# nanoporetech/medaka

Measured on NVIDIA H100. Metric: pileup positions/sec (consensus inference), higher is better.
Workload: dtype f32

## Files before the change

### medaka_b200/csrc/gru_wg.cu

```cuda
#include "common.cuh"
#include "ptx.cuh"
#include "rec_common.cuh"

namespace mdk {

constexpr int RW_THREADS = 256;
constexpr int RW_ABLK = (H / 8) * 64 * 16;
constexpr int RW_XBLK = 2 * 64 * 16;

template <int NT, bool FUSE_X, int OUT>
struct RwCfg {
    static constexpr int N = NT * RT_N;
    static constexpr bool HL = NT == 1;
    static constexpr int ROWS = HL ? 2 * N : N;
    static constexpr int PLANES = HL ? 1 : 2;
    static constexpr int KG = ROWS * 16 + 16;
    static constexpr int HPLANE = (H / 8) * KG;
    static constexpr int XPLANE = 2 * KG;
    static constexpr int HLO = HL ? N * 16 : HPLANE;
    static constexpr int XLO = HL ? N * 16 : XPLANE;
    static constexpr int RED = (RW_THREADS / 32) * NCLS * N;
    static constexpr int wlo_off = 0;
    static constexpr int wxlo_off = wlo_off + 6 * RW_ABLK;
    static constexpr int h_off = wxlo_off + (FUSE_X ? 6 * RW_XBLK : 0);
    static constexpr int x_off = h_off + 2 * PLANES * HPLANE;
    static constexpr int red_off = x_off + (FUSE_X ? 2 * PLANES * XPLANE : 0);
    static constexpr int total = red_off + (OUT == OUT_LOGITS ? 2 * RED * 4 : 0);
    static_assert(total <= 227 * 1024, "smem budget");
};

__device__ __forceinline__ uint32_t ld_u32(const __half *p) { return *reinterpret_cast<const uint32_t *>(p); }

template <int NT, bool FUSE_X, int OUT>
__global__ void __launch_bounds__(RW_THREADS, 1)
rec_tc_kernel(const float *__restrict__ gi, RecX xin, const __half *__restrict__ w_hh, const float *__restrict__ b_hn,
              void *__restrict__ h_out, int64_t B, int64_t T, const float *__restrict__ lin_w,
              float *__restrict__ plog) {
    using L = RwCfg<NT, FUSE_X, OUT>;
    constexpr int N = L::N, NA = N / 2;
    constexpr int NACC = L::ROWS / 2;
    constexpr int NX = FUSE_X ? NACC : NA;
    using MMA = Wgmma<N>;
    using MMA_H = Wgmma<L::ROWS>;
    constexpr bool LOGITS = OUT == OUT_LOGITS;
    extern __shared__ __align__(128) uint8_t smem[];
    const int tid = threadIdx.x, wg = tid >> 7, warp = (tid >> 5) & 3, lane = tid & 31;
    const int gq = lane >> 2, cq = lane & 3;
    const int dir = blockIdx.y;
    const int64_t ntiles = (B + RT_N - 1) / RT_N;
    const int64_t wtile0 = (int64_t)blockIdx.x * NT;
    const int j0 = wg * 64 + warp * 16 + gq;
    const uint32_t sbase = smem_u32(smem);

    for (int i = tid; i < (L::total - L::h_off) / 16; i += RW_THREADS)
        reinterpret_cast<int4 *>(smem + L::h_off)[i] = make_int4(0, 0, 0, 0);
    for (int i = tid; i < 3 * H * (H / 8); i += RW_THREADS) {
        const int kg = i & 15, r = (i >> 4) & (H - 1), gate = i >> 11;
        const uint4 v = *reinterpret_cast<const uint4 *>(w_hh + ((((size_t)dir * 2 + 1) * 3 + gate) * H + r) * H + kg * 8);
        *reinterpret_cast<uint4 *>(smem + L::wlo_off + (gate * 2 + (r >> 6)) * RW_ABLK + kg * 1024 + (r & 63) * 16) = v;
    }
    if (FUSE_X) {
        for (int i = tid; i < 3 * H * 2; i += RW_THREADS) {
            const int kg = i & 1, r = (i >> 1) & (H - 1), gate = i >> 8;
            const uint4 v = *reinterpret_cast<const uint4 *>(xin.w_x + ((((size_t)dir * 2 + 1) * 3 + gate) * H + r) * 16 + kg * 8);
            *reinterpret_cast<uint4 *>(smem + L::wxlo_off + (gate * 2 + (r >> 6)) * RW_XBLK + kg * 1024 + (r & 63) * 16) = v;
        }
    }
    float wlin[2][NCLS];
    if (LOGITS) {
#pragma unroll
        for (int hb = 0; hb < 2; ++hb)
#pragma unroll
            for (int c = 0; c < NCLS; ++c) wlin[hb][c] = lin_w[c * H2 + dir * H + j0 + 8 * hb];
    }
    uint32_t whi[3][H / 16][4];
#pragma unroll
    for (int gate = 0; gate < 3; ++gate)
#pragma unroll
        for (int ks = 0; ks < H / 16; ++ks) {
            const __half *w = w_hh + ((((size_t)dir * 2) * 3 + gate) * H + j0) * H + ks * 16 + 2 * cq;
            whi[gate][ks][0] = ld_u32(w);
            whi[gate][ks][1] = ld_u32(w + 8 * H);
            whi[gate][ks][2] = ld_u32(w + 8);
            whi[gate][ks][3] = ld_u32(w + 8 * H + 8);
        }
    uint32_t wxhi[3][4];
    float bx[3][2] = {};
    if (FUSE_X) {
#pragma unroll
        for (int gate = 0; gate < 3; ++gate) {
            const __half *w = xin.w_x + ((((size_t)dir * 2) * 3 + gate) * H + j0) * 16 + 2 * cq;
            wxhi[gate][0] = ld_u32(w);
            wxhi[gate][1] = ld_u32(w + 8 * 16);
            wxhi[gate][2] = ld_u32(w + 8);
            wxhi[gate][3] = ld_u32(w + 8 * 16 + 8);
            bx[gate][0] = xin.bias[dir * G3 + gate * H + j0];
            bx[gate][1] = xin.bias[dir * G3 + gate * H + j0 + 8];
        }
    }
    const float bhn[2] = {b_hn[dir * H + j0], b_hn[dir * H + j0 + 8]};

    float ar[NACC], az[NACC], an[NACC], axn[NX], hp[NA];
#pragma unroll
    for (int k = 0; k < NA; ++k) hp[k] = 0.f;
    auto load_pre = [&](int64_t t) {
#pragma unroll
        for (int i = 0; i < N / 8; ++i)
#pragma unroll
            for (int hb = 0; hb < 2; ++hb) {
                float2 v[3] = {make_float2(0.f, 0.f), make_float2(0.f, 0.f), make_float2(0.f, 0.f)};
                if (FUSE_X) {
#pragma unroll
                    for (int gate = 0; gate < 3; ++gate) v[gate] = make_float2(bx[gate][hb], bx[gate][hb]);
                } else if (wtile0 + (i >> 1) < ntiles) {
                    const float *p = gi + ((wtile0 + (i >> 1)) * T + t) * GI_TS_FLOATS +
                                     (((dir * 3) * 4 + 2 * (i & 1) + (cq >> 1)) * H + j0 + 8 * hb) * 4 + 2 * (cq & 1);
#pragma unroll
                    for (int gate = 0; gate < 3; ++gate) v[gate] = __ldcs(reinterpret_cast<const float2 *>(p + gate * 16 * H));
                }
                const int k = 4 * i + 2 * hb;
                ar[k] = v[0].x; ar[k + 1] = v[0].y;
                az[k] = v[1].x; az[k + 1] = v[1].y;
                axn[k] = v[2].x; axn[k + 1] = v[2].y;
                an[k] = bhn[hb]; an[k + 1] = bhn[hb];
            }
        if constexpr (L::HL) {
#pragma unroll
            for (int k = NA; k < NACC; ++k) {
                ar[k] = 0.f; az[k] = 0.f; an[k] = 0.f;
                if constexpr (FUSE_X) axn[k] = 0.f;
            }
        }
    };
    const int xF = FUSE_X ? xin.F : 1;
    const float *xsrc[NT];
    int xoff[NT];
    float xreg[NT];
#pragma unroll
    for (int m = 0; m < NT; ++m) {
        const int q = tid + RW_THREADS * m, xn = q / xF, xf = q - xn * xF;
        const bool own = FUSE_X && q < N * xF;
        xoff[m] = own ? (xf >> 3) * L::KG + xn * 16 + (xf & 7) * 2 : -1;
        xsrc[m] = (own && wtile0 * RT_N + xn < B) ? xin.feats + ((wtile0 * RT_N + xn) * T) * xF + xf : nullptr;
        xreg[m] = 0.f;
    }
    auto stage_x = [&](int buf, int m, float v) {
        __half hi, lo;
        split_f16(v, hi, lo);
        *reinterpret_cast<__half *>(smem + L::x_off + buf * L::PLANES * L::XPLANE + xoff[m]) = hi;
        *reinterpret_cast<__half *>(smem + L::x_off + buf * L::PLANES * L::XPLANE + L::XLO + xoff[m]) = lo;
    };
    const int64_t t_first = dir ? T - 1 : 0;
    if (FUSE_X) {
#pragma unroll
        for (int m = 0; m < NT; ++m) {
            if (xoff[m] < 0) continue;
            stage_x(0, m, xsrc[m] ? xsrc[m][t_first * xF] : 0.f);
            if (xsrc[m] && T > 1) xreg[m] = xsrc[m][(dir ? T - 2 : 1) * xF];
        }
    }
    load_pre(t_first);
    fence_proxy_async_smem();
    __syncthreads();

    constexpr int NW = N / 4;
    auto head_partials = [&](int rb) {
        float v[NW][NCLS];
#pragma unroll
        for (int wl = 0; wl < NW; ++wl) {
            const int k = 4 * (wl >> 1) + (wl & 1);
#pragma unroll
            for (int c = 0; c < NCLS; ++c) v[wl][c] = fmaf(wlin[1][c], hp[k + 2], wlin[0][c] * hp[k]);
        }
        int wbase = 0;
#pragma unroll
        for (int lvl = 0; lvl < 3; ++lvl) {
            const int mask = 16 >> lvl;
            const int half = (NW >> lvl) / 2;
            if (half > 0) {
                const bool up = lane & mask;
#pragma unroll
                for (int w = 0; w < NW / 2; ++w) {
                    if (w >= half) continue;
#pragma unroll
                    for (int c = 0; c < NCLS; ++c) {
                        const float send = up ? v[w][c] : v[w + half][c];
                        const float keep = up ? v[w + half][c] : v[w][c];
                        v[w][c] = keep + __shfl_xor_sync(0xffffffffu, send, mask);
                    }
                }
                if (up) wbase += half;
            } else {
#pragma unroll
                for (int c = 0; c < NCLS; ++c) v[0][c] += __shfl_xor_sync(0xffffffffu, v[0][c], mask);
            }
        }
        if (NW >= 8 || !(lane & 4)) {
            float *red = reinterpret_cast<float *>(smem + L::red_off) + rb * L::RED + (tid >> 5) * NCLS * N;
            const int n = 8 * (wbase >> 1) + 2 * cq + (wbase & 1);
#pragma unroll
            for (int c = 0; c < NCLS; ++c) red[c * N + n] = v[0][c];
        }
    };
    auto head_store = [&](int rb, int64_t t) {
        if (tid >= NCLS * N) return;
        const int c = tid / N, n = tid % N;
        const float *red = reinterpret_cast<const float *>(smem + L::red_off) + rb * L::RED + c * N + n;
        float s = red[0];
#pragma unroll
        for (int w = 1; w < RW_THREADS / 32; ++w) s += red[w * NCLS * N];
        const int64_t wt = wtile0 + n / RT_N;
        if (wt < ntiles) plog[((dir * ntiles + wt) * T + t) * PLOG_TS_FLOATS + c * RT_N + (n & 15)] = s;
    };

#pragma unroll 1
    for (int64_t step = 0; step < T; ++step) {
        const int64_t t = dir ? T - 1 - step : step;
        const int buf = (int)(step & 1);
        const uint32_t hb_addr = sbase + L::h_off + buf * L::PLANES * L::HPLANE;
        wg_fence();
        if constexpr (L::HL) {
#pragma unroll
            for (int ks = 0; ks < H / 16; ++ks) {
                const uint64_t bh = make_smem_desc(hb_addr + ks * 2 * L::KG, L::KG, 128);
#pragma unroll
                for (int gate = 0; gate < 3; ++gate) MMA_H::rs(gate == 0 ? ar : (gate == 1 ? az : an), whi[gate][ks], bh, 1u);
#pragma unroll
                for (int gate = 0; gate < 3; ++gate)
                    MMA::ss(gate == 0 ? ar : (gate == 1 ? az : an),
                            make_smem_desc(sbase + L::wlo_off + (gate * 2 + wg) * RW_ABLK + ks * 2 * 1024, 1024, 128), bh, 1u);
            }
        } else {
#pragma unroll
            for (int gate = 0; gate < 3; ++gate) {
                float(&acc)[NACC] = gate == 0 ? ar : (gate == 1 ? az : an);
#pragma unroll
                for (int ks = 0; ks < H / 16; ++ks) {
                    const uint64_t bh = make_smem_desc(hb_addr + ks * 2 * L::KG, L::KG, 128);
                    MMA::rs(acc, whi[gate][ks], bh, 1u);
                    MMA::rs(acc, whi[gate][ks], make_smem_desc(hb_addr + L::HPLANE + ks * 2 * L::KG, L::KG, 128), 1u);
                    MMA::ss(acc, make_smem_desc(sbase + L::wlo_off + (gate * 2 + wg) * RW_ABLK + ks * 2 * 1024, 1024, 128), bh, 1u);
                }
            }
        }
        if constexpr (FUSE_X) {
            const uint32_t xa = sbase + L::x_off + buf * L::PLANES * L::XPLANE;
            const uint64_t bh = make_smem_desc(xa, L::KG, 128);
            if constexpr (L::HL) {
#pragma unroll
                for (int gate = 0; gate < 3; ++gate) MMA_H::rs(gate == 0 ? ar : (gate == 1 ? az : axn), wxhi[gate], bh, 1u);
#pragma unroll
                for (int gate = 0; gate < 3; ++gate)
                    MMA::ss(gate == 0 ? ar : (gate == 1 ? az : axn),
                            make_smem_desc(sbase + L::wxlo_off + (gate * 2 + wg) * RW_XBLK, 1024, 128), bh, 1u);
            } else {
                const uint64_t bl = make_smem_desc(xa + L::XPLANE, L::KG, 128);
#pragma unroll
                for (int gate = 0; gate < 3; ++gate) {
                    float(&acc)[NACC] = gate == 0 ? ar : (gate == 1 ? az : axn);
                    MMA::rs(acc, wxhi[gate], bh, 1u);
                    MMA::rs(acc, wxhi[gate], bl, 1u);
                    MMA::ss(acc, make_smem_desc(sbase + L::wxlo_off + (gate * 2 + wg) * RW_XBLK, 1024, 128), bh, 1u);
                }
            }
        }
        wg_commit();
        if (!FUSE_X && tid == 0 && step + GI_PREFETCH_STEPS < T) {
            const int64_t tp = dir ? t - GI_PREFETCH_STEPS : t + GI_PREFETCH_STEPS;
#pragma unroll
            for (int m = 0; m < NT; ++m) {
                if (wtile0 + m >= ntiles) break;
                const float *blk = gi + ((wtile0 + m) * T + tp) * GI_TS_FLOATS + (int64_t)dir * (GI_TS_FLOATS / 2);
#pragma unroll
                for (int i = 0; i < 12; ++i) bulk_prefetch_l2(blk + i * 512, 2048);
            }
        }
        if (LOGITS && step > 0) {
            if (step > 1) head_store((int)((step - 1) & 1), dir ? t + 2 : t - 2);
            head_partials((int)(step & 1));
        }
        wg_wait_all();
        wg_hold(ar); wg_hold(az); wg_hold(an); wg_hold(axn);

        uint8_t *hw = smem + L::h_off + (buf ^ 1) * L::PLANES * L::HPLANE;
#pragma unroll
        for (int k = 0; k < NA; ++k) {
            float pr = ar[k], pz = az[k], pn = an[k], px = axn[k], r, z;
            if constexpr (L::HL) {
                pr += ar[k + NA]; pz += az[k + NA]; pn += an[k + NA];
                if constexpr (FUSE_X) px += axn[k + NA];
                const float a = 1.f + ex2_approx(fminf(pr, EXP_CLAMP)), b = 1.f + ex2_approx(fminf(pz, EXP_CLAMP));
                const float q = rcp_approx(a * b);
                r = b * q;
                z = a * q;
            } else {
                r = rcp_approx(1.f + ex2_approx(fminf(pr, EXP_CLAMP)));
                z = rcp_approx(1.f + ex2_approx(fminf(pz, EXP_CLAMP)));
            }
            const float en = ex2_approx(fminf(fmaf(r, pn, px), EXP_CLAMP));
            const float n = (en - 1.f) * rcp_approx(en + 1.f);
            hp[k] = fmaf(z, hp[k] - n, n);
            const int j = j0 + 8 * ((k >> 1) & 1), col = 8 * (k >> 2) + 2 * cq + (k & 1);
            __half hi, lo;
            split_f16(hp[k], hi, lo);
            *reinterpret_cast<__half *>(hw + (j >> 3) * L::KG + col * 16 + (j & 7) * 2) = hi;
            *reinterpret_cast<__half *>(hw + L::HLO + (j >> 3) * L::KG + col * 16 + (j & 7) * 2) = lo;
        }
        if (FUSE_X && step + 1 < T) {
#pragma unroll
            for (int m = 0; m < NT; ++m) {
                if (xoff[m] < 0) continue;
                stage_x(buf ^ 1, m, xreg[m]);
                if (xsrc[m] && step + 2 < T) xreg[m] = xsrc[m][(dir ? t - 2 : t + 2) * xF];
            }
        }
        if (!LOGITS) {
#pragma unroll
            for (int k = 0; k < NA; ++k) {
                const int i = k >> 2, n = 8 * i + 2 * cq + (k & 1);
                const int64_t wt = wtile0 + (i >> 1);
                if (wt >= ntiles) continue;
                const int64_t orow = (wt * T + t) * RT_N + (n & 15);
                const int kcol = dir * H + j0 + 8 * ((k >> 1) & 1);
                if (OUT == OUT_TILES) {
                    __half hi, lo;
                    split_f16(hp[k], hi, lo);
                    __half *o = reinterpret_cast<__half *>(reinterpret_cast<uint8_t *>(h_out) + (orow >> 7) * (int64_t)XT_TILE_BYTES +
                                                           (kcol >> 3) * (XT_ROWS * 16) + (orow & (XT_ROWS - 1)) * 16) + (kcol & 7);
                    o[0] = hi;
                    o[XT_PLANE_BYTES / 2] = lo;
                } else {
                    reinterpret_cast<float *>(h_out)[orow * H2 + kcol] = hp[k];
                }
            }
        }
        if (step + 1 < T) load_pre(dir ? t - 1 : t + 1);
        fence_proxy_async_smem();
        __syncthreads();
    }
    if (LOGITS) {
        if (T > 1) head_store((int)((T - 1) & 1), dir ? 1 : T - 2);
        head_partials((int)(T & 1));
        __syncthreads();
        head_store((int)(T & 1), dir ? 0 : T - 1);
    }
}

template <int NT, bool FX, int OUT>
static cudaError_t launch_rec(const float *gi, const RecX &xin, const __half *w_hh_tm, const float *b_hn, void *out,
                              const float *lin_w, int64_t B, int64_t T, cudaStream_t s) {
    auto kern = rec_tc_kernel<NT, FX, OUT>;
    constexpr int smem_bytes = RwCfg<NT, FX, OUT>::total;
    cudaError_t e = cudaFuncSetAttribute(kern, cudaFuncAttributeMaxDynamicSharedMemorySize, smem_bytes);
    if (e != cudaSuccess) return e;
    const int64_t tiles = (B + RT_N - 1) / RT_N;
    dim3 grid((unsigned)((tiles + NT - 1) / NT), NDIR);
    constexpr bool LOGITS = OUT == OUT_LOGITS;
    kern<<<grid, RW_THREADS, smem_bytes, s>>>(gi, xin, w_hh_tm, b_hn, LOGITS ? nullptr : out, B, T, lin_w,
                                              LOGITS ? static_cast<float *>(out) : nullptr);
    return cudaGetLastError();
}

template <int NT>
static cudaError_t launch_rec_nt(const float *gi, const RecX *xin, const __half *w_hh_tm, const float *b_hn, int out_kind,
                                 void *out, const float *lin_w, int64_t B, int64_t T, cudaStream_t s) {
    if (xin)
        return out_kind == OUT_TILES ? launch_rec<NT, true, OUT_TILES>(gi, *xin, w_hh_tm, b_hn, out, nullptr, B, T, s)
                                     : cudaErrorInvalidValue;
    const RecX none{nullptr, nullptr, nullptr, 0};
    switch (out_kind) {
    case OUT_TILES: return launch_rec<NT, false, OUT_TILES>(gi, none, w_hh_tm, b_hn, out, nullptr, B, T, s);
    case OUT_ROWS: return launch_rec<NT, false, OUT_ROWS>(gi, none, w_hh_tm, b_hn, out, nullptr, B, T, s);
    case OUT_LOGITS:
        return lin_w ? launch_rec<NT, false, OUT_LOGITS>(gi, none, w_hh_tm, b_hn, out, lin_w, B, T, s) : cudaErrorInvalidValue;
    }
    return cudaErrorInvalidValue;
}

cudaError_t launch_rec_tc(const float *gi, const RecX *xin, const __half *w_hh_tm, const float *b_hn, int tiles_per_cta,
                          int out_kind, void *out, const float *lin_w, int64_t B, int64_t T, cudaStream_t s) {
    if (B == 0 || T == 0) return cudaSuccess;
    switch (tiles_per_cta) {
    case 1: return launch_rec_nt<1>(gi, xin, w_hh_tm, b_hn, out_kind, out, lin_w, B, T, s);
    case 2: return launch_rec_nt<2>(gi, xin, w_hh_tm, b_hn, out_kind, out, lin_w, B, T, s);
    }
    return cudaErrorInvalidValue;
}

constexpr int GW_THREADS = 256;
constexpr int GW_QK = 8;
constexpr int GW_STAGE_PLANE = GW_QK * XT_ROWS * 16;
constexpr int GW_STAGE = 2 * GW_STAGE_PLANE;
constexpr int GW_NQ = XT_K / 8 / GW_QK;
constexpr int GW_X_OFF = XT_TILE_BYTES;
constexpr int GW_BAR_OFF = GW_X_OFF + 2 * GW_STAGE;
constexpr int GW_SMEM = GW_BAR_OFF + 16;

__global__ void __launch_bounds__(GW_THREADS, 1)
gemm_tc_kernel(const uint8_t *__restrict__ x_tiles, const __half *__restrict__ w_in_tm, const float *__restrict__ bias,
               float *__restrict__ gi, int64_t P, int64_t ntiles) {
    extern __shared__ __align__(128) uint8_t smem[];
    uint64_t *full = reinterpret_cast<uint64_t *>(smem + GW_BAR_OFF);
    const int tid = threadIdx.x, wg = tid >> 7, warp = (tid >> 5) & 3, lane = tid & 31;
    const int gq = lane >> 2, cq = lane & 3;
    const int blk = blockIdx.x;
    const uint32_t sbase = smem_u32(smem);
    for (int i = tid; i < 2 * H * (H2 / 8); i += GW_THREADS) {
        const int kg = i & 31, r = (i >> 5) & (H - 1), p = i >> 12;
        const uint4 v = reinterpret_cast<const uint4 *>(w_in_tm + (((size_t)blk * 2 + p) * H + r) * H2)[kg];
        *reinterpret_cast<uint4 *>(smem + p * XT_PLANE_BYTES + kg * (XT_ROWS * 16) + r * 16) = v;
    }
    if (tid == 0) {
        mbar_init(&full[0], 1);
        mbar_init(&full[1], 1);
        fence_mbar_init();
    }
    fence_proxy_async_smem();
    __syncthreads();
    const int64_t my_tiles = blockIdx.y < ntiles ? (ntiles - 1 - blockIdx.y) / gridDim.y + 1 : 0;
    const int64_t nst = my_tiles * GW_NQ;
    auto issue = [&](int64_t it) {
        const int64_t tile = blockIdx.y + (it / GW_NQ) * gridDim.y;
        const int q = (int)(it % GW_NQ), s = (int)(it & 1);
        const uint8_t *src = x_tiles + tile * (int64_t)XT_TILE_BYTES + q * GW_STAGE_PLANE;
        mbar_arrive_expect_tx(&full[s], GW_STAGE);
        bulk_g2s(smem + GW_X_OFF + s * GW_STAGE, src, GW_STAGE_PLANE, &full[s]);
        bulk_g2s(smem + GW_X_OFF + s * GW_STAGE + GW_STAGE_PLANE, src + XT_PLANE_BYTES, GW_STAGE_PLANE, &full[s]);
    };
    if (tid == 0) {
        if (nst > 0) issue(0);
        if (nst > 1) issue(1);
    }
    const float bj[2] = {bias[blk * H + wg * 64 + warp * 16 + gq], bias[blk * H + wg * 64 + warp * 16 + gq + 8]};
    float acc[64];
#pragma unroll 1
    for (int64_t it = 0; it < nst; ++it) {
        const int q = (int)(it % GW_NQ), s = (int)(it & 1);
        mbar_wait(&full[s], (uint32_t)((it >> 1) & 1));
        wg_fence();
#pragma unroll
        for (int prod = 0; prod < 3; ++prod) {
            const int pa = prod == 2, pb = prod == 1;
#pragma unroll
            for (int kk = 0; kk < GW_QK / 2; ++kk) {
                const uint64_t a = make_smem_desc(sbase + pa * XT_PLANE_BYTES + (q * GW_QK + 2 * kk) * (XT_ROWS * 16) + wg * 64 * 16,
                                                  XT_ROWS * 16, 128);
                const uint64_t b = make_smem_desc(sbase + GW_X_OFF + s * GW_STAGE + pb * GW_STAGE_PLANE + 2 * kk * (XT_ROWS * 16),
                                                  XT_ROWS * 16, 128);
                Wgmma<128>::ss(acc, a, b, (q | prod | kk) ? 1u : 0u);
            }
        }
        wg_commit();
        wg_wait_all();
        wg_hold(acc);
        __syncthreads();
        if (tid == 0 && it + 2 < nst) issue(it + 2);
        if (q == GW_NQ - 1) {
            const int64_t tile = blockIdx.y + (it / GW_NQ) * gridDim.y;
            const int64_t prem = P - tile * XT_ROWS;
#pragma unroll
            for (int k = 0; k < 64; k += 2) {
                const int c = 8 * (k >> 2) + 2 * cq, hb = (k >> 1) & 1;
                if (c >= prem) continue;
                const int j = wg * 64 + warp * 16 + gq + 8 * hb;
                float *o = gi + ((((tile * (XT_ROWS / WT) + (c >> 4)) * 6 + blk) * 4 + ((c & 15) >> 2)) * H + j) * 4 + (c & 3);
                __stcs(reinterpret_cast<float2 *>(o), make_float2(acc[k] + bj[hb], acc[k + 1] + bj[hb]));
            }
        }
    }
}

cudaError_t launch_gemm_tc(const void *x_tiles, const __half *w_in_tm, const float *bias, float *gi, int64_t P,
                           int sm_count, cudaStream_t s) {
    if (P == 0) return cudaSuccess;
    const int64_t ntiles = (P + XT_ROWS - 1) / XT_ROWS;
    cudaError_t ea = cudaFuncSetAttribute(gemm_tc_kernel, cudaFuncAttributeMaxDynamicSharedMemorySize, GW_SMEM);
    if (ea != cudaSuccess) return ea;
    int64_t ct = sm_count / 6;
    if (ct < 1) ct = 1;
    if (ct > ntiles) ct = ntiles;
    dim3 grid(6, (unsigned)ct);
    gemm_tc_kernel<<<grid, GW_THREADS, GW_SMEM, s>>>(reinterpret_cast<const uint8_t *>(x_tiles), w_in_tm, bias, gi, P, ntiles);
    return cudaGetLastError();
}

__global__ void __launch_bounds__(256, 1)
selftest_kernel(const float *__restrict__ A, const float *__restrict__ Bm, float *__restrict__ D, int N, int K) {
    extern __shared__ __align__(128) uint8_t smem[];
    const int a_plane = 128 * K * 2, b_plane = N * K * 2;
    uint8_t *sa = smem, *sb = smem + 2 * a_plane;
    const int tid = threadIdx.x, wg = tid >> 7, warp = (tid >> 5) & 3, lane = tid & 31;
    for (int i = tid; i < 128 * K; i += 256) {
        const int r = i / K, k = i % K;
        __half hi, lo;
        split_f16(A[i], hi, lo);
        const int off = (k / 8) * (128 * 16) + r * 16 + (k % 8) * 2;
        *reinterpret_cast<__half *>(sa + off) = hi;
        *reinterpret_cast<__half *>(sa + a_plane + off) = lo;
    }
    for (int i = tid; i < N * K; i += 256) {
        const int r = i / K, k = i % K;
        __half hi, lo;
        split_f16(Bm[i], hi, lo);
        const int off = (k / 8) * (N * 16) + r * 16 + (k % 8) * 2;
        *reinterpret_cast<__half *>(sb + off) = hi;
        *reinterpret_cast<__half *>(sb + b_plane + off) = lo;
    }
    fence_proxy_async_smem();
    __syncthreads();
    for (int n0 = 0; n0 < N; n0 += 16) {
        float d[8];
        wg_fence();
        uint32_t acc = 0;
        for (int prod = 0; prod < 3; ++prod) {
            const int pa = (prod == 2), pb = (prod == 1);
            for (int ks = 0; ks < K / 16; ++ks) {
                const uint64_t ad = make_smem_desc(smem_u32(sa + pa * a_plane) + ks * 2 * 128 * 16 + wg * 64 * 16, 128 * 16, 128);
                const uint64_t bd = make_smem_desc(smem_u32(sb + pb * b_plane) + ks * 2 * N * 16 + n0 * 16, N * 16, 128);
                Wgmma<16>::ss(d, ad, bd, acc);
                acc = 1;
            }
        }
        wg_commit();
        wg_wait_all();
        wg_hold(d);
        const int row = wg * 64 + warp * 16 + (lane >> 2);
        for (int k = 0; k < 8; ++k)
            D[(row + 8 * ((k >> 1) & 1)) * N + n0 + 8 * (k >> 2) + 2 * (lane & 3) + (k & 1)] = d[k];
    }
}

int selftest_umma(int device, const float *A, const float *B, float *D, int N, int K, int variant) {
    MDK_REQUIRE(N >= 16 && N <= 128 && N % 16 == 0, MDK_ERR_ARG, "selftest_umma: N must be a multiple of 16 in [16,128]");
    MDK_REQUIRE(K >= 16 && K <= 256 && K % 16 == 0, MDK_ERR_ARG, "selftest_umma: K must be a multiple of 16 in [16,256]");
    MDK_REQUIRE(variant == 0, MDK_ERR_ARG, "selftest_umma: variant must be 0");
    MDK_CUDA(cudaSetDevice(device));
    float *dA = nullptr, *dB = nullptr, *dD = nullptr;
    MDK_CUDA(cudaMalloc(&dA, sizeof(float) * 128 * K));
    MDK_CUDA(cudaMalloc(&dB, sizeof(float) * N * K));
    MDK_CUDA(cudaMalloc(&dD, sizeof(float) * 128 * N));
    MDK_CUDA(cudaMemcpy(dA, A, sizeof(float) * 128 * K, cudaMemcpyHostToDevice));
    MDK_CUDA(cudaMemcpy(dB, B, sizeof(float) * N * K, cudaMemcpyHostToDevice));
    const int smem = 2 * 128 * K * 2 + 2 * N * K * 2;
    MDK_REQUIRE(smem <= 227 * 1024, MDK_ERR_ARG, "selftest_umma: N*K too large for shared memory");
    MDK_CUDA(cudaFuncSetAttribute(selftest_kernel, cudaFuncAttributeMaxDynamicSharedMemorySize, smem));
    selftest_kernel<<<1, 256, smem>>>(dA, dB, dD, N, K);
    MDK_CUDA(cudaGetLastError());
    MDK_CUDA(cudaDeviceSynchronize());
    MDK_CUDA(cudaMemcpy(D, dD, sizeof(float) * 128 * N, cudaMemcpyDeviceToHost));
    cudaFree(dA); cudaFree(dB); cudaFree(dD);
    return MDK_OK;
}

}
```

### medaka_b200/csrc/ptx.cuh

```cuda
#pragma once
#include <cstdint>
#include <cuda_fp16.h>

namespace mdk {

__device__ __forceinline__ uint32_t smem_u32(const void *p) {
    return static_cast<uint32_t>(__cvta_generic_to_shared(p));
}

__device__ __forceinline__ void mbar_init(uint64_t *bar, uint32_t count) {
    asm volatile("mbarrier.init.shared::cta.b64 [%0], %1;" ::"r"(smem_u32(bar)), "r"(count) : "memory");
}
__device__ __forceinline__ void fence_mbar_init() {
    asm volatile("fence.mbarrier_init.release.cluster;" ::: "memory");
}
__device__ __forceinline__ void mbar_arrive_expect_tx(uint64_t *bar, uint32_t bytes) {
    asm volatile("mbarrier.arrive.expect_tx.shared::cta.b64 _, [%0], %1;" ::"r"(smem_u32(bar)), "r"(bytes)
                 : "memory");
}
__device__ __forceinline__ bool mbar_try_wait(uint64_t *bar, uint32_t parity) {
    uint32_t ok;
    asm volatile(
        "{\n\t.reg .pred p;\n\t"
        "mbarrier.try_wait.parity.shared::cta.b64 p, [%1], %2;\n\t"
        "selp.u32 %0, 1, 0, p;\n\t}"
        : "=r"(ok)
        : "r"(smem_u32(bar)), "r"(parity)
        : "memory");
    return ok != 0;
}
__device__ __forceinline__ void mbar_wait(uint64_t *bar, uint32_t parity) {
    if (mbar_try_wait(bar, parity)) return;
    const long long t0 = clock64();
    while (!mbar_try_wait(bar, parity)) {
        if (clock64() - t0 > 4000000000LL) __trap();
    }
}

__device__ __forceinline__ void fence_proxy_async_smem() {
    asm volatile("fence.proxy.async.shared::cta;" ::: "memory");
}

__device__ __forceinline__ uint32_t cluster_ctarank() {
    uint32_t r;
    asm volatile("mov.u32 %0, %%cluster_ctarank;" : "=r"(r));
    return r;
}
__device__ __forceinline__ uint32_t mapa_shared(uint32_t smem_addr, uint32_t rank) {
    uint32_t r;
    asm volatile("mapa.shared::cluster.u32 %0, %1, %2;" : "=r"(r) : "r"(smem_addr), "r"(rank));
    return r;
}
__device__ __forceinline__ void st_cluster_u32(uint32_t cluster_addr, uint32_t v) {
    asm volatile("st.shared::cluster.u32 [%0], %1;" ::"r"(cluster_addr), "r"(v) : "memory");
}
__device__ __forceinline__ void fence_proxy_async_cluster() {
    asm volatile("fence.proxy.async.shared::cluster;" ::: "memory");
}
__device__ __forceinline__ void mbar_arrive_cluster(uint32_t cluster_addr) {
    asm volatile("mbarrier.arrive.release.cluster.shared::cluster.b64 _, [%0];" ::"r"(cluster_addr) : "memory");
}
__device__ __forceinline__ bool mbar_try_wait_cluster(uint64_t *bar, uint32_t parity) {
    uint32_t ok;
    asm volatile(
        "{\n\t.reg .pred p;\n\t"
        "mbarrier.try_wait.parity.acquire.cluster.shared::cta.b64 p, [%1], %2;\n\t"
        "selp.u32 %0, 1, 0, p;\n\t}"
        : "=r"(ok)
        : "r"(smem_u32(bar)), "r"(parity)
        : "memory");
    return ok != 0;
}
__device__ __forceinline__ void mbar_wait_cluster(uint64_t *bar, uint32_t parity) {
    if (mbar_try_wait_cluster(bar, parity)) return;
    const long long t0 = clock64();
    while (!mbar_try_wait_cluster(bar, parity)) {
        if (clock64() - t0 > 4000000000LL) __trap();
    }
}
__device__ __forceinline__ void cluster_sync_all() {
    asm volatile("barrier.cluster.arrive.release.aligned;\n\tbarrier.cluster.wait.acquire.aligned;" ::: "memory");
}
__device__ __forceinline__ void named_bar_sync(uint32_t id, uint32_t count) {
    asm volatile("bar.sync %0, %1;" ::"r"(id), "r"(count) : "memory");
}

__device__ __forceinline__ void bulk_prefetch_l2(const void *gmem_src, uint32_t bytes) {
    asm volatile("cp.async.bulk.prefetch.L2.global [%0], %1;" ::"l"(gmem_src), "r"(bytes) : "memory");
}

__device__ __forceinline__ void bulk_g2s(void *smem_dst, const void *gmem_src, uint32_t bytes, uint64_t *bar) {
    asm volatile(
        "cp.async.bulk.shared::cluster.global.mbarrier::complete_tx::bytes [%0], [%1], %2, [%3];" ::"r"(
            smem_u32(smem_dst)),
        "l"(gmem_src), "r"(bytes), "r"(smem_u32(bar))
        : "memory");
}

__device__ __forceinline__ uint64_t make_smem_desc(uint32_t smem_addr, uint32_t lbo_bytes, uint32_t sbo_bytes) {
    uint64_t d = 0;
    d |= static_cast<uint64_t>((smem_addr & 0x3FFFF) >> 4);
    d |= static_cast<uint64_t>((lbo_bytes >> 4) & 0x3FFF) << 16;
    d |= static_cast<uint64_t>((sbo_bytes >> 4) & 0x3FFF) << 32;
    return d;
}
__device__ __forceinline__ void wg_fence() { asm volatile("wgmma.fence.sync.aligned;" ::: "memory"); }
__device__ __forceinline__ void wg_commit() { asm volatile("wgmma.commit_group.sync.aligned;" ::: "memory"); }
__device__ __forceinline__ void wg_wait_all() { asm volatile("wgmma.wait_group.sync.aligned 0;" ::: "memory"); }
template <int R>
__device__ __forceinline__ void wg_hold(float (&d)[R]) {
#pragma unroll
    for (int i = 0; i < R; ++i) asm volatile("" : "+f"(d[i])::"memory");
}

template <int N> struct Wgmma;
template <> struct Wgmma<16> {
    __device__ __forceinline__ static void ss(float (&d)[8], uint64_t a, uint64_t b, uint32_t accumulate) {
        asm volatile(
            "{\n\t.reg .pred p;\n\tsetp.ne.b32 p, %10, 0;\n\t"
            "wgmma.mma_async.sync.aligned.m64n16k16.f32.f16.f16 {%0,%1,%2,%3,%4,%5,%6,%7}, %8, %9, p, 1, 1, 0, 0;\n\t}"
            : "+f"(d[0]), "+f"(d[1]), "+f"(d[2]), "+f"(d[3]), "+f"(d[4]), "+f"(d[5]), "+f"(d[6]), "+f"(d[7])
            : "l"(a), "l"(b), "r"(accumulate));
    }
    __device__ __forceinline__ static void rs(float (&d)[8], const uint32_t (&a)[4], uint64_t b, uint32_t accumulate) {
        asm volatile(
            "{\n\t.reg .pred p;\n\tsetp.ne.b32 p, %13, 0;\n\t"
            "wgmma.mma_async.sync.aligned.m64n16k16.f32.f16.f16 {%0,%1,%2,%3,%4,%5,%6,%7}, {%8,%9,%10,%11}, %12, p, 1, 1, 0;\n\t}"
            : "+f"(d[0]), "+f"(d[1]), "+f"(d[2]), "+f"(d[3]), "+f"(d[4]), "+f"(d[5]), "+f"(d[6]), "+f"(d[7])
            : "r"(a[0]), "r"(a[1]), "r"(a[2]), "r"(a[3]), "l"(b), "r"(accumulate));
    }
    __device__ __forceinline__ static void ss(float (&d)[16], uint64_t a, uint64_t b, uint32_t accumulate) {
        asm volatile(
            "{\n\t.reg .pred p;\n\tsetp.ne.b32 p, %10, 0;\n\t"
            "wgmma.mma_async.sync.aligned.m64n16k16.f32.f16.f16 {%0,%1,%2,%3,%4,%5,%6,%7}, %8, %9, p, 1, 1, 0, 0;\n\t}"
            : "+f"(d[0]), "+f"(d[1]), "+f"(d[2]), "+f"(d[3]), "+f"(d[4]), "+f"(d[5]), "+f"(d[6]), "+f"(d[7])
            : "l"(a), "l"(b), "r"(accumulate));
    }
};
template <> struct Wgmma<32> {
    __device__ __forceinline__ static void ss(float (&d)[16], uint64_t a, uint64_t b, uint32_t accumulate) {
        asm volatile(
            "{\n\t.reg .pred p;\n\tsetp.ne.b32 p, %18, 0;\n\t"
            "wgmma.mma_async.sync.aligned.m64n32k16.f32.f16.f16 {%0,%1,%2,%3,%4,%5,%6,%7,%8,%9,%10,%11,%12,%13,%14,%15}, %16, %17, p, 1, 1, 0, 0;\n\t}"
            : "+f"(d[0]), "+f"(d[1]), "+f"(d[2]), "+f"(d[3]), "+f"(d[4]), "+f"(d[5]), "+f"(d[6]), "+f"(d[7]),
              "+f"(d[8]), "+f"(d[9]), "+f"(d[10]), "+f"(d[11]), "+f"(d[12]), "+f"(d[13]), "+f"(d[14]), "+f"(d[15])
            : "l"(a), "l"(b), "r"(accumulate));
    }
    __device__ __forceinline__ static void rs(float (&d)[16], const uint32_t (&a)[4], uint64_t b, uint32_t accumulate) {
        asm volatile(
            "{\n\t.reg .pred p;\n\tsetp.ne.b32 p, %21, 0;\n\t"
            "wgmma.mma_async.sync.aligned.m64n32k16.f32.f16.f16 {%0,%1,%2,%3,%4,%5,%6,%7,%8,%9,%10,%11,%12,%13,%14,%15}, {%16,%17,%18,%19}, %20, p, 1, 1, 0;\n\t}"
            : "+f"(d[0]), "+f"(d[1]), "+f"(d[2]), "+f"(d[3]), "+f"(d[4]), "+f"(d[5]), "+f"(d[6]), "+f"(d[7]),
              "+f"(d[8]), "+f"(d[9]), "+f"(d[10]), "+f"(d[11]), "+f"(d[12]), "+f"(d[13]), "+f"(d[14]), "+f"(d[15])
            : "r"(a[0]), "r"(a[1]), "r"(a[2]), "r"(a[3]), "l"(b), "r"(accumulate));
    }
};
template <> struct Wgmma<128> {
    __device__ __forceinline__ static void ss(float (&d)[64], uint64_t a, uint64_t b, uint32_t accumulate) {
        asm volatile(
            "{\n\t.reg .pred p;\n\tsetp.ne.b32 p, %66, 0;\n\t"
            "wgmma.mma_async.sync.aligned.m64n128k16.f32.f16.f16 {%0,%1,%2,%3,%4,%5,%6,%7,%8,%9,%10,%11,%12,%13,%14,%15,%16,%17,%18,%19,%20,%21,%22,%23,%24,%25,%26,%27,%28,%29,%30,%31,%32,%33,%34,%35,%36,%37,%38,%39,%40,%41,%42,%43,%44,%45,%46,%47,%48,%49,%50,%51,%52,%53,%54,%55,%56,%57,%58,%59,%60,%61,%62,%63}, %64, %65, p, 1, 1, 0, 0;\n\t}"
            : "+f"(d[0]), "+f"(d[1]), "+f"(d[2]), "+f"(d[3]), "+f"(d[4]), "+f"(d[5]), "+f"(d[6]), "+f"(d[7]),
              "+f"(d[8]), "+f"(d[9]), "+f"(d[10]), "+f"(d[11]), "+f"(d[12]), "+f"(d[13]), "+f"(d[14]), "+f"(d[15]),
              "+f"(d[16]), "+f"(d[17]), "+f"(d[18]), "+f"(d[19]), "+f"(d[20]), "+f"(d[21]), "+f"(d[22]), "+f"(d[23]),
              "+f"(d[24]), "+f"(d[25]), "+f"(d[26]), "+f"(d[27]), "+f"(d[28]), "+f"(d[29]), "+f"(d[30]), "+f"(d[31]),
              "+f"(d[32]), "+f"(d[33]), "+f"(d[34]), "+f"(d[35]), "+f"(d[36]), "+f"(d[37]), "+f"(d[38]), "+f"(d[39]),
              "+f"(d[40]), "+f"(d[41]), "+f"(d[42]), "+f"(d[43]), "+f"(d[44]), "+f"(d[45]), "+f"(d[46]), "+f"(d[47]),
              "+f"(d[48]), "+f"(d[49]), "+f"(d[50]), "+f"(d[51]), "+f"(d[52]), "+f"(d[53]), "+f"(d[54]), "+f"(d[55]),
              "+f"(d[56]), "+f"(d[57]), "+f"(d[58]), "+f"(d[59]), "+f"(d[60]), "+f"(d[61]), "+f"(d[62]), "+f"(d[63])
            : "l"(a), "l"(b), "r"(accumulate));
    }
};

__host__ __device__ __forceinline__ void split_f16(float v, __half &hi, __half &lo) {
    hi = __float2half_rn(v);
    lo = __float2half_rn(v - __half2float(hi));
}

__device__ __forceinline__ float ldg_stream(const float *p) {
    float v;
    asm volatile("ld.global.nc.L1::no_allocate.f32 %0, [%1];" : "=f"(v) : "l"(p));
    return v;
}

__device__ __forceinline__ float4 ld_stream4(const float *p) {
    float4 v;
    asm volatile("ld.global.nc.L1::no_allocate.v4.f32 {%0,%1,%2,%3}, [%4];"
                 : "=f"(v.x), "=f"(v.y), "=f"(v.z), "=f"(v.w)
                 : "l"(p));
    return v;
}

}
```

Before: 155.4 million.

## Pipeline input-projection GEMM with register-resident weights and TMA bulk stores

The input-projection GEMM kernel now keeps the weight A-operand in registers and issues register-sourced wgmma, which frees shared memory. It buffers every K-stage of an X tile using per-stage full/empty mbarriers, so the next tile's loads overlap the current compute. Results are staged in padded shared memory and written with per-lane bulk shared-to-global copies carrying an L2 evict-first hint, replacing scattered streaming float2 stores. This adds register pressure (wa array plus 64 accumulators) and extra syncs per tile, and the epilogue now depends on correct bulk-store fencing.

```diff
diff --git a/medaka_b200/csrc/gru_wg.cu b/medaka_b200/csrc/gru_wg.cu
--- a/medaka_b200/csrc/gru_wg.cu
+++ b/medaka_b200/csrc/gru_wg.cu
@@ -392,82 +392,113 @@
 constexpr int GW_STAGE_PLANE = GW_QK * XT_ROWS * 16;
 constexpr int GW_STAGE = 2 * GW_STAGE_PLANE;
 constexpr int GW_NQ = XT_K / 8 / GW_QK;
-constexpr int GW_X_OFF = XT_TILE_BYTES;
-constexpr int GW_BAR_OFF = GW_X_OFF + 2 * GW_STAGE;
-constexpr int GW_SMEM = GW_BAR_OFF + 16;
+constexpr int GW_KS = XT_K / 16;
+constexpr int GW_TS = XT_ROWS / WT;
+constexpr int GW_QUAD = H * 4;
+constexpr int GW_QUAD_PAD = GW_QUAD + 16;
+constexpr int GW_OUT_OFF = GW_NQ * GW_STAGE;
+constexpr int GW_BAR_OFF = GW_OUT_OFF + GW_TS * 4 * GW_QUAD_PAD * 4;
+constexpr int GW_SMEM = GW_BAR_OFF + 2 * GW_NQ * 8;
+static_assert(GW_SMEM <= 227 * 1024, "smem budget");
+static_assert(GW_TS * 4 == 32, "one bulk store per lane of warp 0");
 
 __global__ void __launch_bounds__(GW_THREADS, 1)
 gemm_tc_kernel(const uint8_t *__restrict__ x_tiles, const __half *__restrict__ w_in_tm, const float *__restrict__ bias,
                float *__restrict__ gi, int64_t P, int64_t ntiles) {
     extern __shared__ __align__(128) uint8_t smem[];
-    uint64_t *full = reinterpret_cast<uint64_t *>(smem + GW_BAR_OFF);
+    uint64_t *full = reinterpret_cast<uint64_t *>(smem + GW_BAR_OFF), *empty = full + GW_NQ;
+    float *stg = reinterpret_cast<float *>(smem + GW_OUT_OFF);
     const int tid = threadIdx.x, wg = tid >> 7, warp = (tid >> 5) & 3, lane = tid & 31;
     const int gq = lane >> 2, cq = lane & 3;
     const int blk = blockIdx.x;
+    const int j0 = wg * 64 + warp * 16 + gq;
     const uint32_t sbase = smem_u32(smem);
-    for (int i = tid; i < 2 * H * (H2 / 8); i += GW_THREADS) {
-        const int kg = i & 31, r = (i >> 5) & (H - 1), p = i >> 12;
-        const uint4 v = reinterpret_cast<const uint4 *>(w_in_tm + (((size_t)blk * 2 + p) * H + r) * H2)[kg];
-        *reinterpret_cast<uint4 *>(smem + p * XT_PLANE_BYTES + kg * (XT_ROWS * 16) + r * 16) = v;
-    }
-    if (tid == 0) {
-        mbar_init(&full[0], 1);
-        mbar_init(&full[1], 1);
-        fence_mbar_init();
-    }
-    fence_proxy_async_smem();
-    __syncthreads();
     const int64_t my_tiles = blockIdx.y < ntiles ? (ntiles - 1 - blockIdx.y) / gridDim.y + 1 : 0;
-    const int64_t nst = my_tiles * GW_NQ;
-    auto issue = [&](int64_t it) {
-        const int64_t tile = blockIdx.y + (it / GW_NQ) * gridDim.y;
-        const int q = (int)(it % GW_NQ), s = (int)(it & 1);
-        const uint8_t *src = x_tiles + tile * (int64_t)XT_TILE_BYTES + q * GW_STAGE_PLANE;
-        mbar_arrive_expect_tx(&full[s], GW_STAGE);
-        bulk_g2s(smem + GW_X_OFF + s * GW_STAGE, src, GW_STAGE_PLANE, &full[s]);
-        bulk_g2s(smem + GW_X_OFF + s * GW_STAGE + GW_STAGE_PLANE, src + XT_PLANE_BYTES, GW_STAGE_PLANE, &full[s]);
+    auto issue = [&](int64_t n, int q) {
+        const uint8_t *src = x_tiles + (blockIdx.y + n * gridDim.y) * (int64_t)XT_TILE_BYTES + q * GW_STAGE_PLANE;
+        mbar_arrive_expect_tx(&full[q], GW_STAGE);
+        bulk_g2s(smem + q * GW_STAGE, src, GW_STAGE_PLANE, &full[q]);
+        bulk_g2s(smem + q * GW_STAGE + GW_STAGE_PLANE, src + XT_PLANE_BYTES, GW_STAGE_PLANE, &full[q]);
     };
     if (tid == 0) {
-        if (nst > 0) issue(0);
-        if (nst > 1) issue(1);
-    }
-    const float bj[2] = {bias[blk * H + wg * 64 + warp * 16 + gq], bias[blk * H + wg * 64 + warp * 16 + gq + 8]};
+        for (int q = 0; q < GW_NQ; ++q) {
+            mbar_init(&full[q], 1);
+            mbar_init(&empty[q], GW_THREADS / 32);
+        }
+        fence_mbar_init();
+        if (my_tiles > 0)
+            for (int q = 0; q < GW_NQ; ++q) issue(0, q);
+    }
+    uint32_t wa[2][GW_KS][4];
+#pragma unroll
+    for (int p = 0; p < 2; ++p)
+#pragma unroll
+        for (int ks = 0; ks < GW_KS; ++ks) {
+            const __half *w = w_in_tm + (((size_t)blk * 2 + p) * H + j0) * H2 + ks * 16 + 2 * cq;
+            wa[p][ks][0] = ld_u32(w);
+            wa[p][ks][1] = ld_u32(w + 8 * H2);
+            wa[p][ks][2] = ld_u32(w + 8);
+            wa[p][ks][3] = ld_u32(w + 8 * H2 + 8);
+        }
+    const float bj[2] = {bias[blk * H + j0], bias[blk * H + j0 + 8]};
+    const uint64_t policy = l2_evict_first_policy();
+    __syncthreads();
+    auto release = [&](int64_t n, int q) {
+        if (lane == 0) mbar_arrive(&empty[q]);
+        if (tid == 0 && n + 1 < my_tiles) {
+            mbar_wait(&empty[q], (uint32_t)(n & 1));
+            issue(n + 1, q);
+        }
+        __syncwarp();
+    };
     float acc[64];
 #pragma unroll 1
-    for (int64_t it = 0; it < nst; ++it) {
-        const int q = (int)(it % GW_NQ), s = (int)(it & 1);
-        mbar_wait(&full[s], (uint32_t)((it >> 1) & 1));
-        wg_fence();
-#pragma unroll
-        for (int prod = 0; prod < 3; ++prod) {
-            const int pa = prod == 2, pb = prod == 1;
-#pragma unroll
-            for (int kk = 0; kk < GW_QK / 2; ++kk) {
-                const uint64_t a = make_smem_desc(sbase + pa * XT_PLANE_BYTES + (q * GW_QK + 2 * kk) * (XT_ROWS * 16) + wg * 64 * 16,
-                                                  XT_ROWS * 16, 128);
-                const uint64_t b = make_smem_desc(sbase + GW_X_OFF + s * GW_STAGE + pb * GW_STAGE_PLANE + 2 * kk * (XT_ROWS * 16),
-                                                  XT_ROWS * 16, 128);
-                Wgmma<128>::ss(acc, a, b, (q | prod | kk) ? 1u : 0u);
-            }
-        }
-        wg_commit();
+    for (int64_t n = 0; n < my_tiles; ++n) {
+#pragma unroll
+        for (int q = 0; q < GW_NQ; ++q) {
+            mbar_wait(&full[q], (uint32_t)(n & 1));
+            wg_fence();
+#pragma unroll
+            for (int prod = 0; prod < 3; ++prod) {
+                const int pa = prod == 2, pb = prod == 1;
+#pragma unroll
+                for (int kk = 0; kk < GW_QK / 2; ++kk) {
+                    const uint64_t b = make_smem_desc(sbase + q * GW_STAGE + pb * GW_STAGE_PLANE + 2 * kk * (XT_ROWS * 16),
+                                                      XT_ROWS * 16, 128);
+                    Wgmma<128>::rs(acc, wa[pa][q * (GW_QK / 2) + kk], b, (q | prod | kk) ? 1u : 0u);
+                }
+            }
+            wg_commit();
+            if (q > 0) {
+                wg_wait_1();
+                release(n, q - 1);
+            }
+        }
         wg_wait_all();
         wg_hold(acc);
+        release(n, GW_NQ - 1);
+
+        const int64_t tile = blockIdx.y + n * gridDim.y;
+        const int64_t prem = P - tile * XT_ROWS;
+        if (tid < 32) bulk_wait_read_all();
         __syncthreads();
-        if (tid == 0 && it + 2 < nst) issue(it + 2);
-        if (q == GW_NQ - 1) {
-            const int64_t tile = blockIdx.y + (it / GW_NQ) * gridDim.y;
-            const int64_t prem = P - tile * XT_ROWS;
-#pragma unroll
-            for (int k = 0; k < 64; k += 2) {
-                const int c = 8 * (k >> 2) + 2 * cq, hb = (k >> 1) & 1;
-                if (c >= prem) continue;
-                const int j = wg * 64 + warp * 16 + gq + 8 * hb;
-                float *o = gi + ((((tile * (XT_ROWS / WT) + (c >> 4)) * 6 + blk) * 4 + ((c & 15) >> 2)) * H + j) * 4 + (c & 3);
-                __stcs(reinterpret_cast<float2 *>(o), make_float2(acc[k] + bj[hb], acc[k + 1] + bj[hb]));
-            }
-        }
-    }
+#pragma unroll
+        for (int k = 0; k < 64; k += 2) {
+            const int i = k >> 2, hb = (k >> 1) & 1;
+            float *o = stg + ((i >> 1) * 4 + 2 * (i & 1) + (cq >> 1)) * GW_QUAD_PAD + (j0 + 8 * hb) * 4 + 2 * (cq & 1);
+            *reinterpret_cast<float2 *>(o) = make_float2(acc[k] + bj[hb], acc[k + 1] + bj[hb]);
+        }
+        fence_proxy_async_smem();
+        __syncthreads();
+        if (tid < 32) {
+            const int ts = lane >> 2, cg = lane & 3;
+            if (ts * WT < prem)
+                bulk_s2g(gi + (((tile * GW_TS + ts) * 6 + blk) * 4 + cg) * GW_QUAD, stg + lane * GW_QUAD_PAD,
+                         GW_QUAD * 4, policy);
+            bulk_commit();
+        }
+    }
+    if (tid < 32) bulk_wait_all();
 }
 
 cudaError_t launch_gemm_tc(const void *x_tiles, const __half *w_in_tm, const float *bias, float *gi, int64_t P,
diff --git a/medaka_b200/csrc/ptx.cuh b/medaka_b200/csrc/ptx.cuh
--- a/medaka_b200/csrc/ptx.cuh
+++ b/medaka_b200/csrc/ptx.cuh
@@ -17,6 +17,9 @@
 __device__ __forceinline__ void mbar_arrive_expect_tx(uint64_t *bar, uint32_t bytes) {
     asm volatile("mbarrier.arrive.expect_tx.shared::cta.b64 _, [%0], %1;" ::"r"(smem_u32(bar)), "r"(bytes)
                  : "memory");
+}
+__device__ __forceinline__ void mbar_arrive(uint64_t *bar) {
+    asm volatile("mbarrier.arrive.shared::cta.b64 _, [%0];" ::"r"(smem_u32(bar)) : "memory");
 }
 __device__ __forceinline__ bool mbar_try_wait(uint64_t *bar, uint32_t parity) {
     uint32_t ok;
@@ -96,6 +99,19 @@
         "l"(gmem_src), "r"(bytes), "r"(smem_u32(bar))
         : "memory");
 }
+__device__ __forceinline__ uint64_t l2_evict_first_policy() {
+    uint64_t p;
+    asm volatile("createpolicy.fractional.L2::evict_first.b64 %0, 1.0;" : "=l"(p));
+    return p;
+}
+__device__ __forceinline__ void bulk_s2g(void *gmem_dst, const void *smem_src, uint32_t bytes, uint64_t policy) {
+    asm volatile("cp.async.bulk.global.shared::cta.bulk_group.L2::cache_hint [%0], [%1], %2, %3;" ::"l"(gmem_dst),
+                 "r"(smem_u32(smem_src)), "r"(bytes), "l"(policy)
+                 : "memory");
+}
+__device__ __forceinline__ void bulk_commit() { asm volatile("cp.async.bulk.commit_group;" ::: "memory"); }
+__device__ __forceinline__ void bulk_wait_read_all() { asm volatile("cp.async.bulk.wait_group.read 0;" ::: "memory"); }
+__device__ __forceinline__ void bulk_wait_all() { asm volatile("cp.async.bulk.wait_group 0;" ::: "memory"); }
 
 __device__ __forceinline__ uint64_t make_smem_desc(uint32_t smem_addr, uint32_t lbo_bytes, uint32_t sbo_bytes) {
     uint64_t d = 0;
@@ -107,6 +123,7 @@
 __device__ __forceinline__ void wg_fence() { asm volatile("wgmma.fence.sync.aligned;" ::: "memory"); }
 __device__ __forceinline__ void wg_commit() { asm volatile("wgmma.commit_group.sync.aligned;" ::: "memory"); }
 __device__ __forceinline__ void wg_wait_all() { asm volatile("wgmma.wait_group.sync.aligned 0;" ::: "memory"); }
+__device__ __forceinline__ void wg_wait_1() { asm volatile("wgmma.wait_group.sync.aligned 1;" ::: "memory"); }
 template <int R>
 __device__ __forceinline__ void wg_hold(float (&d)[R]) {
 #pragma unroll
@@ -170,6 +187,20 @@
               "+f"(d[56]), "+f"(d[57]), "+f"(d[58]), "+f"(d[59]), "+f"(d[60]), "+f"(d[61]), "+f"(d[62]), "+f"(d[63])
             : "l"(a), "l"(b), "r"(accumulate));
     }
+    __device__ __forceinline__ static void rs(float (&d)[64], const uint32_t (&a)[4], uint64_t b, uint32_t accumulate) {
+        asm volatile(
+            "{\n\t.reg .pred p;\n\tsetp.ne.b32 p, %69, 0;\n\t"
+            "wgmma.mma_async.sync.aligned.m64n128k16.f32.f16.f16 {%0,%1,%2,%3,%4,%5,%6,%7,%8,%9,%10,%11,%12,%13,%14,%15,%16,%17,%18,%19,%20,%21,%22,%23,%24,%25,%26,%27,%28,%29,%30,%31,%32,%33,%34,%35,%36,%37,%38,%39,%40,%41,%42,%43,%44,%45,%46,%47,%48,%49,%50,%51,%52,%53,%54,%55,%56,%57,%58,%59,%60,%61,%62,%63}, {%64,%65,%66,%67}, %68, p, 1, 1, 0;\n\t}"
+            : "+f"(d[0]), "+f"(d[1]), "+f"(d[2]), "+f"(d[3]), "+f"(d[4]), "+f"(d[5]), "+f"(d[6]), "+f"(d[7]),
+              "+f"(d[8]), "+f"(d[9]), "+f"(d[10]), "+f"(d[11]), "+f"(d[12]), "+f"(d[13]), "+f"(d[14]), "+f"(d[15]),
+              "+f"(d[16]), "+f"(d[17]), "+f"(d[18]), "+f"(d[19]), "+f"(d[20]), "+f"(d[21]), "+f"(d[22]), "+f"(d[23]),
+              "+f"(d[24]), "+f"(d[25]), "+f"(d[26]), "+f"(d[27]), "+f"(d[28]), "+f"(d[29]), "+f"(d[30]), "+f"(d[31]),
+              "+f"(d[32]), "+f"(d[33]), "+f"(d[34]), "+f"(d[35]), "+f"(d[36]), "+f"(d[37]), "+f"(d[38]), "+f"(d[39]),
+              "+f"(d[40]), "+f"(d[41]), "+f"(d[42]), "+f"(d[43]), "+f"(d[44]), "+f"(d[45]), "+f"(d[46]), "+f"(d[47]),
+              "+f"(d[48]), "+f"(d[49]), "+f"(d[50]), "+f"(d[51]), "+f"(d[52]), "+f"(d[53]), "+f"(d[54]), "+f"(d[55]),
+              "+f"(d[56]), "+f"(d[57]), "+f"(d[58]), "+f"(d[59]), "+f"(d[60]), "+f"(d[61]), "+f"(d[62]), "+f"(d[63])
+            : "r"(a[0]), "r"(a[1]), "r"(a[2]), "r"(a[3]), "l"(b), "r"(accumulate));
+    }
 };
 
 __host__ __device__ __forceinline__ void split_f16(float v, __half &hi, __half &lo) {
```

New measurement: 163.9 million (median of 6 runs). 5.5% higher.
